# EloDoyard/movie-recommender-system

Hardware: AMD Instinct MI355X
Metric: test-set predictions/sec (kNN k=300, fit+predict+MAE) (higher is better)
Workload: dtype fp16 MFMA similarity filter (fp32 acc) + f64 exact re-rank/prediction

## Files before the change

### movie-recommender-system_amd/csrc/gemm.hip

```cpp
#include <algorithm>
#include <type_traits>
#include <vector>

#include "engine.h"
#include "wave_helpers.h"

namespace knncf {

typedef __attribute__((ext_vector_type(8))) __bf16 bf16x8;
typedef __attribute__((ext_vector_type(8))) _Float16 f16x8;
typedef __attribute__((ext_vector_type(16))) float f32x16;

template <bool F16>
__global__ void k_densify(const int64_t* __restrict__ u_ptr, const int32_t* __restrict__ s_col,
                          const double* __restrict__ s_pre, const int32_t* __restrict__ rows, int32_t row_begin,
                          int32_t n_rows, const int32_t* __restrict__ colmap, bf16_t* __restrict__ panel, int64_t ld, int ones) {
    int32_t wave = (blockIdx.x * blockDim.x + threadIdx.x) >> 6;
    int32_t lane = threadIdx.x & 63;
    if (wave >= n_rows) return;
    int32_t u = rows ? rows[wave] : row_begin + wave;
    int64_t b = u_ptr[u], e = u_ptr[u + 1];
    bf16_t* out = panel + (int64_t)wave * ld;
    for (int64_t p = b + lane; p < e; p += 64) {
        int32_t c = colmap ? colmap[s_col[p]] : s_col[p];
        if (c >= 0) {
            const float x = ones ? 1.0f : (float)s_pre[p];
            if (F16) reinterpret_cast<_Float16*>(out)[c] = (_Float16)x;
            else out[c] = (bf16_t)x;
        }
    }
}

template <bool F16>
__global__ void __launch_bounds__(256) k_densify_rows(const int64_t* __restrict__ u_ptr, const int32_t* __restrict__ s_col,
                                                      const double* __restrict__ s_pre, const int32_t* __restrict__ rows, int32_t row_begin,
                                                      int32_t n_rows, const int32_t* __restrict__ colmap, bf16_t* __restrict__ panel, int64_t ld,
                                                      int ones) {
    extern __shared__ __attribute__((aligned(16))) char smem[];
    const int lane = threadIdx.x & 63;
    const int32_t n_waves = (int32_t)((gridDim.x * blockDim.x) >> 6);
    bf16_t* my = reinterpret_cast<bf16_t*>(smem) + (size_t)(threadIdx.x >> 6) * ld;
    auto wave_sync = [] {
        __builtin_amdgcn_fence(__ATOMIC_ACQ_REL, "wavefront");
        __builtin_amdgcn_wave_barrier();
    };
    for (int32_t wave = (int32_t)((blockIdx.x * blockDim.x + threadIdx.x) >> 6); wave < n_rows; wave += n_waves) {
        for (int64_t c = lane; c < ld / 8; c += 64) reinterpret_cast<uint4*>(my)[c] = make_uint4(0u, 0u, 0u, 0u);
        wave_sync();
        const int32_t u = rows ? rows[wave] : row_begin + wave;
        const int64_t b = u_ptr[u], e = u_ptr[u + 1];
        for (int64_t p0 = b; p0 < e; p0 += 512) {
            int32_t it[8];
            double xv[8];
            int32_t cc[8];
#pragma unroll
            for (int q = 0; q < 8; ++q) {
                const int64_t p = p0 + 64 * q + lane;
                it[q] = p < e ? s_col[p] : -1;
                xv[q] = (p < e && !ones) ? s_pre[p] : 1.0;
            }
#pragma unroll
            for (int q = 0; q < 8; ++q) cc[q] = it[q] < 0 ? -1 : (colmap ? colmap[it[q]] : it[q]);
#pragma unroll
            for (int q = 0; q < 8; ++q) {
                if (cc[q] >= 0) {
                    if (F16) reinterpret_cast<_Float16*>(my)[cc[q]] = (_Float16)(float)xv[q];
                    else my[cc[q]] = (bf16_t)(float)xv[q];
                }
            }
        }
        wave_sync();
        uint4* out = reinterpret_cast<uint4*>(panel + (int64_t)wave * ld);
        for (int64_t c = lane; c < ld / 8; c += 64) out[c] = reinterpret_cast<const uint4*>(my)[c];
        wave_sync();
    }
}

void launch_densify(const Train& tr, const int32_t* d_rows, int32_t row_begin, int32_t n_rows,
                    const int32_t* d_colmap, bf16_t* panel, int64_t ld, int64_t panel_rows, bool fp16, hipStream_t st) {
    const size_t lds = (size_t)4 * (size_t)ld * sizeof(bf16_t);
    if (ld % 64 == 0 && lds <= 64 * 1024) {
        if (panel_rows > n_rows) KN_HIP(hipMemsetAsync(panel + (int64_t)n_rows * ld, 0, (size_t)(panel_rows - n_rows) * ld * sizeof(bf16_t), st));
        if (n_rows <= 0) return;
        const int blocks = (int)std::min<int64_t>(ceil_div((int64_t)n_rows * 64, 256), 256 * 16);
        if (fp16) k_densify_rows<true><<<blocks, 256, lds, st>>>(tr.u_ptr.p, tr.s_col.p, tr.s_pre.p, d_rows, row_begin, n_rows, d_colmap, panel, ld, tr.jaccard ? 1 : 0);
        else k_densify_rows<false><<<blocks, 256, lds, st>>>(tr.u_ptr.p, tr.s_col.p, tr.s_pre.p, d_rows, row_begin, n_rows, d_colmap, panel, ld, tr.jaccard ? 1 : 0);
        KN_HIP(hipGetLastError());
        return;
    }
    KN_HIP(hipMemsetAsync(panel, 0, (size_t)panel_rows * ld * sizeof(bf16_t), st));
    if (n_rows <= 0) return;
    int blocks = (int)ceil_div((int64_t)n_rows * 64, 256);
    if (fp16) k_densify<true><<<blocks, 256, 0, st>>>(tr.u_ptr.p, tr.s_col.p, tr.s_pre.p, d_rows, row_begin, n_rows, d_colmap, panel, ld, tr.jaccard ? 1 : 0);
    else k_densify<false><<<blocks, 256, 0, st>>>(tr.u_ptr.p, tr.s_col.p, tr.s_pre.p, d_rows, row_begin, n_rows, d_colmap, panel, ld, tr.jaccard ? 1 : 0);
    KN_HIP(hipGetLastError());
}

__global__ void k_colmap(int32_t I, int32_t H, const int32_t* __restrict__ pop_item, int32_t* __restrict__ colmap) {
    int32_t j = blockIdx.x * blockDim.x + threadIdx.x;
    if (j >= I) return;
    colmap[pop_item[j]] = j < H ? j : -1;
}

void launch_colmap(const Train& tr, int32_t H, int32_t* d_colmap, hipStream_t st) {
    k_colmap<<<(unsigned)ceil_div(tr.I, 256), 256, 0, st>>>(tr.I, H, tr.pop_item.p, d_colmap);
    KN_HIP(hipGetLastError());
}

static constexpr int BK = 64;

template <int ROWS>
struct TileGeom {
    static constexpr int TILE_BYTES = ROWS * BK * 2;
    static constexpr int STAGE_BYTES = 2 * TILE_BYTES;
};

template <int ROWS, int WAVES>
__device__ __forceinline__ void stage_tile(const bf16_t* __restrict__ g, int64_t ld, char* lds_tile, int wave, int lane) {
    constexpr int LOADS = ROWS / 8 / WAVES;
#pragma unroll
    for (int j = 0; j < LOADS; ++j) {
        int piece = wave * LOADS + j;
        int row = piece * 8 + (lane >> 3);
        int slot = lane & 7;
        int chunk = slot ^ ((row >> 1) & 7);
        const bf16_t* src = g + (int64_t)row * ld + chunk * 8;
        __builtin_amdgcn_global_load_lds(src, (__attribute__((address_space(3))) void*)(lds_tile + piece * 1024), 16, 0, 0);
    }
}

__device__ __forceinline__ bf16x8 read_frag(const char* lds_tile, int row, int chunk) {
    int slot = chunk ^ ((row >> 1) & 7);
    return *reinterpret_cast<const bf16x8*>(lds_tile + row * 128 + slot * 16);
}

template <bool F16>
__device__ __forceinline__ f32x16 mfma(bf16x8 a, bf16x8 b, f32x16 c) {
    if (F16) return __builtin_amdgcn_mfma_f32_32x32x16_f16(__builtin_bit_cast(f16x8, a), __builtin_bit_cast(f16x8, b), c, 0, 0, 0);
    return __builtin_amdgcn_mfma_f32_32x32x16_bf16(a, b, c, 0, 0, 0);
}

struct EpiGeom {
    static constexpr int WM = 4, WN = 2, WAVES_M = 2, WAVES_N = 4, TB = 256;
    static constexpr int ESZ = (int)sizeof(float);
    static constexpr int IPP = WM / 2;
    static constexpr int PASS_ROWS = IPP * 32;
    static constexpr int PASSES = WAVES_M * (WM / IPP);
    static constexpr int RS = TB * ESZ + 16;
    static constexpr int IMAGE_N = PASS_ROWS * RS;
    static constexpr int RS_T = PASS_ROWS * ESZ + 16;
    static constexpr int IMAGE_T = TB * RS_T;
    static constexpr int IMAGE = IMAGE_N > IMAGE_T ? IMAGE_N : IMAGE_T;
    static constexpr int STAGE = TileGeom<TB>::STAGE_BYTES;
    static constexpr int PAD = IMAGE > STAGE ? ((IMAGE - STAGE + 1023) / 1024) * 1024 : 0;
    static constexpr int SMEM = 2 * STAGE + 2 * PAD;
};

template <bool F16, bool SYM>
__global__ void __launch_bounds__(EpiGeom::WAVES_M * EpiGeom::WAVES_N * 64)
k_gemm_nt_bf16(const bf16_t* __restrict__ A, const bf16_t* __restrict__ B, float* __restrict__ C, int tiles_m,
               int tiles_n, int k_tiles, int64_t lda, int64_t ldb, int64_t ldc, const uint32_t* __restrict__ tile_list, int n_listed) {
    typedef EpiGeom EG;
    constexpr int WM = EG::WM, WN = EG::WN, WAVES_N = EG::WAVES_N, WAVES = EG::WAVES_M * EG::WAVES_N, TB = EG::TB;
    constexpr int TILE_BYTES = TileGeom<TB>::TILE_BYTES, STAGE_BYTES = TileGeom<TB>::STAGE_BYTES;
    constexpr int LOADS_PER_STAGE = 2 * (TB / 8 / WAVES);
    static_assert(LOADS_PER_STAGE == 8, "the counted vmcnt below assumes 8 LDS-DMA instructions per wave per stage");
    extern __shared__ __attribute__((aligned(1024))) char lds[];
    char* const ring = lds + EG::PAD;

    const int nwg = SYM ? n_listed : tiles_m * tiles_n;
    const int xcd = blockIdx.x & 7, q = nwg >> 3, r = nwg & 7;
    const int xcd_first = xcd < r ? xcd * (q + 1) : r * (q + 1) + (xcd - r) * q;
    const int xcd_end = xcd_first + (xcd < r ? q + 1 : q);
    const int stride = ((int)gridDim.x - xcd + 7) >> 3;
    int t = xcd_first + ((int)blockIdx.x >> 3);
    if (t >= xcd_end) return;

    const int lane = threadIdx.x & 63;
    const int wave = threadIdx.x >> 6;
    const int wr = wave / WAVES_N, wc = wave % WAVES_N;
    const int frow = lane & 31;
    const int fhalf = lane >> 5;

    auto tile_of = [&](int wg, int& tm, int& tn) {
        if (SYM) {
            const uint32_t packed = tile_list[wg];
            tm = (int)(packed & 0xffffu);
            tn = (int)(packed >> 16);
            return;
        }
        const int GROUP = 8;
        const int group_sz = GROUP * tiles_n;
        const int gid = wg / group_sz;
        const int first_m = gid * GROUP;
        const int gm = min(GROUP, tiles_m - first_m);
        tm = first_m + (wg % group_sz) % gm;
        tn = (wg % group_sz) / gm;
    };

    int tm, tn;
    tile_of(t, tm, tn);
    const bf16_t* Ag = A + (int64_t)tm * TB * lda;
    const bf16_t* Bg = B + (int64_t)tn * TB * ldb;
    stage_tile<TB, WAVES>(Ag, lda, ring, wave, lane);
    stage_tile<TB, WAVES>(Bg, ldb, ring + TILE_BYTES, wave, lane);
    int slot = 0;
    bool landed = false;

    for (;;) {
        const int t_next = t + stride;
        const bool more = t_next < xcd_end;
        int tm2 = 0, tn2 = 0;
        if (more) tile_of(t_next, tm2, tn2);
        const bf16_t* Ag2 = A + (int64_t)tm2 * TB * lda;
        const bf16_t* Bg2 = B + (int64_t)tn2 * TB * ldb;

        f32x16 acc[WM][WN];
#pragma unroll
        for (int i = 0; i < WM; ++i)
#pragma unroll
            for (int j = 0; j < WN; ++j)
#pragma unroll
                for (int e = 0; e < 16; ++e) acc[i][j][e] = 0.f;

        for (int kt = 0; kt < k_tiles; ++kt) {
            char* cur = ring + slot * STAGE_BYTES;
            char* nxt = ring + (slot ^ 1) * STAGE_BYTES;
            const bool in_tile = kt + 1 < k_tiles;
            if (in_tile) {
                stage_tile<TB, WAVES>(Ag + (int64_t)(kt + 1) * BK, lda, nxt, wave, lane);
                stage_tile<TB, WAVES>(Bg + (int64_t)(kt + 1) * BK, ldb, nxt + TILE_BYTES, wave, lane);
            } else if (more) {
                stage_tile<TB, WAVES>(Ag2, lda, nxt, wave, lane);
                stage_tile<TB, WAVES>(Bg2, ldb, nxt + TILE_BYTES, wave, lane);
            }
            if (!landed) {
                if (in_tile || more) asm volatile("s_waitcnt vmcnt(8)" ::: "memory");
                else asm volatile("s_waitcnt vmcnt(0)" ::: "memory");
            }
            landed = false;
            __builtin_amdgcn_s_barrier();
            asm volatile("" ::: "memory");
#pragma unroll
            for (int ks = 0; ks < BK / 16; ++ks) {
                bf16x8 a[WM];
#pragma unroll
                for (int i = 0; i < WM; ++i) a[i] = read_frag(cur, wr * (WM * 32) + i * 32 + frow, ks * 2 + fhalf);
                bf16x8 b[WN];
#pragma unroll
                for (int j = 0; j < WN; ++j) b[j] = read_frag(cur + TILE_BYTES, wc * (WN * 32) + j * 32 + frow, ks * 2 + fhalf);
#pragma unroll
                for (int i = 0; i < WM; ++i)
#pragma unroll
                    for (int j = 0; j < WN; ++j)
                        acc[i][j] = mfma<F16>(b[j], a[i], acc[i][j]);
            }
            asm volatile("s_waitcnt lgkmcnt(0)" ::: "memory");
            __builtin_amdgcn_s_barrier();
            asm volatile("" ::: "memory");
            slot ^= 1;
        }

        {
            asm volatile("s_waitcnt vmcnt(0)" ::: "memory");
            landed = more;
            constexpr int ESZ = EG::ESZ, RS = EG::RS, IPP = EG::IPP, PASS_ROWS = EG::PASS_ROWS, PASSES = EG::PASSES;
            constexpr int CH = TB * ESZ / 16;
            char* const img = (slot ^ 1) ? ring + STAGE_BYTES : lds;
#pragma unroll
            for (int pass = 0; pass < PASSES; ++pass) {
                const int wrp = pass / (WM / IPP), i0 = (pass % (WM / IPP)) * IPP;
                if (wr == wrp) {
#pragma unroll
                    for (int ii = 0; ii < IPP; ++ii)
#pragma unroll
                        for (int j = 0; j < WN; ++j)
#pragma unroll
                            for (int g = 0; g < 4; ++g) {
                                const int i = i0 + ii;
                                char* dst = img + (ii * 32 + frow) * RS + (wc * (WN * 32) + j * 32 + 8 * g + 4 * fhalf) * ESZ;
                                *reinterpret_cast<float4*>(dst) = make_float4(acc[i][j][4 * g], acc[i][j][4 * g + 1], acc[i][j][4 * g + 2], acc[i][j][4 * g + 3]);
                            }
                }
                __syncthreads();
                float* Cg = C + ((int64_t)tm * TB + wrp * (WM * 32) + i0 * 32) * ldc + (int64_t)tn * TB;
                for (int idx = threadIdx.x; idx < PASS_ROWS * CH; idx += WAVES * 64) {
                    const int row = idx / CH, ch = idx - row * CH;
                    const uint4 v = *reinterpret_cast<const uint4*>(img + row * RS + ch * 16);
                    typedef __attribute__((ext_vector_type(4))) uint32_t u32x4;
                    __builtin_nontemporal_store(__builtin_bit_cast(u32x4, v), reinterpret_cast<u32x4*>(reinterpret_cast<char*>(Cg + (int64_t)row * ldc) + ch * 16));
                }
                __syncthreads();
                if (SYM && tm != tn) {
                    constexpr int RS_T = EG::RS_T;
                    constexpr int CHT = PASS_ROWS * ESZ / 16;
                    if (wr == wrp) {
#pragma unroll
                        for (int ii = 0; ii < IPP; ++ii)
#pragma unroll
                            for (int j = 0; j < WN; ++j)
#pragma unroll
                                for (int g = 0; g < 4; ++g)
#pragma unroll
                                    for (int e = 0; e < 4; ++e) {
                                        const int i = i0 + ii;
                                        const int col = wc * (WN * 32) + j * 32 + 8 * g + 4 * fhalf + e;
                                        float* dst = reinterpret_cast<float*>(img + col * RS_T) + (ii * 32 + frow);
                                        *dst = acc[i][j][4 * g + e];
                                    }
                    }
                    __syncthreads();
                    float* Ct = C + (int64_t)tn * TB * ldc + (int64_t)tm * TB + wrp * (WM * 32) + i0 * 32;
                    for (int idx = threadIdx.x; idx < TB * CHT; idx += WAVES * 64) {
                        const int row = idx / CHT, ch = idx - row * CHT;
                        const uint4 v = *reinterpret_cast<const uint4*>(img + row * RS_T + ch * 16);
                        typedef __attribute__((ext_vector_type(4))) uint32_t u32x4;
                        __builtin_nontemporal_store(__builtin_bit_cast(u32x4, v), reinterpret_cast<u32x4*>(reinterpret_cast<char*>(Ct + (int64_t)row * ldc) + ch * 16));
                    }
                    __syncthreads();
                }
            }
        }
        if (!more) break;
        t = t_next;
        tm = tm2;
        tn = tn2;
        Ag = Ag2;
        Bg = Bg2;
    }
}

template <int ROWS, int WAVES>
__device__ __forceinline__ void stage_tile_u(const bf16_t* g_uniform, uint32_t ld2, char* lds_tile, int wave, uint32_t voff) {
    constexpr int LOADS = ROWS / 8 / WAVES;
    static_assert(LOADS % 2 == 0, "pieces alternate between even and odd");
    const char* base = reinterpret_cast<const char*>(uniform_ptr(g_uniform));
#ifdef KNNCF_OV_ABL_NOLOAD
    return;
#endif
#pragma unroll
    for (int j = 0; j < LOADS; ++j) {
        const int piece = wave * LOADS + j;
        const char* src = base + (uint64_t)((uint32_t)piece * 8u * ld2) + (uint64_t)((j & 1) ? (voff ^ 64u) : voff);
        __builtin_amdgcn_global_load_lds(reinterpret_cast<const bf16_t*>(src), (__attribute__((address_space(3))) void*)(lds_tile + piece * 1024), 16, 0, 0);
    }
}

#ifdef KNNCF_OV_ABL_NOSTORE
#define KN_OV_STORE "s_nop 0 ; "
#define KN_OV_STORES 0
#else
#define KN_OV_STORE
#define KN_OV_STORES 4
#endif
template <bool F16, bool SYM, bool SPREAD>
__global__ void __launch_bounds__(512)
k_gemm_nt_ov(const bf16_t* __restrict__ A, const bf16_t* __restrict__ B, _Float16* __restrict__ C, int tiles_m, int tiles_n,
             int k_tiles, int64_t lda, int64_t ldb, int64_t ldc, const uint32_t* __restrict__ tile_list, int n_listed, float clamp_hi) {
    constexpr int WM = 4, WN = 2, WAVES_N = 4, WAVES = 8, TB = 256;
    constexpr int TILE_BYTES = TileGeom<TB>::TILE_BYTES, STAGE_BYTES = TileGeom<TB>::STAGE_BYTES;
    constexpr int LOADS_PER_STAGE = 2 * (TB / 8 / WAVES);
    static_assert(LOADS_PER_STAGE == 8, "the counted waits below assume 8 LDS-DMA instructions per wave per stage");
    extern __shared__ __attribute__((aligned(1024))) char lds[];
    char* const ring = lds;

    const int nwg = SYM ? n_listed : tiles_m * tiles_n;
    const int xcd = blockIdx.x & 7, q = nwg >> 3, r = nwg & 7;
    const int xcd_first = xcd < r ? xcd * (q + 1) : r * (q + 1) + (xcd - r) * q;
    const int xcd_end = xcd_first + (xcd < r ? q + 1 : q);
    const int stride = ((int)gridDim.x - xcd + 7) >> 3;
    int t = xcd_first + ((int)blockIdx.x >> 3);
    if (t >= xcd_end) return;

    const int lane = threadIdx.x & 63;
    const int wave = threadIdx.x >> 6;
    const int wr = wave / WAVES_N, wc = wave % WAVES_N;
    const int frow = lane & 31, fhalf = lane >> 5;
    char* const stg = lds + 2 * STAGE_BYTES + wave * 4096;
    const int uwave = __builtin_amdgcn_readfirstlane(wave);
    const uint32_t lda2 = (uint32_t)lda * 2u, ldb2 = (uint32_t)ldb * 2u;
    const uint32_t sw16 = (uint32_t)(((lane & 7) ^ (lane >> 4)) * 16);
    uint32_t voff_a = (uint32_t)(lane >> 3) * lda2 + sw16, voff_b = (uint32_t)(lane >> 3) * ldb2 + sw16;
    asm volatile("" : "+v"(voff_a), "+v"(voff_b));

    auto tile_of = [&](int wg, int& tm, int& tn) {
        if (SYM) {
            const uint32_t packed = tile_list[wg];
            tm = (int)(packed & 0xffffu);
            tn = (int)(packed >> 16);
            return;
        }
        const int GROUP = 8;
        const int group_sz = GROUP * tiles_n;
        const int gid = wg / group_sz;
        const int first_m = gid * GROUP;
        const int gm = min(GROUP, tiles_m - first_m);
        tm = first_m + (wg % group_sz) % gm;
        tn = (wg % group_sz) / gm;
    };

    typedef __attribute__((ext_vector_type(2))) _Float16 h2;
    typedef __attribute__((ext_vector_type(4))) uint32_t u32x4;
    constexpr int NP = 2, UNITS = 4;
    uint32_t P[NP][WN][8];
#pragma unroll
    for (int i = 0; i < NP; ++i)
#pragma unroll
        for (int j = 0; j < WN; ++j)
#pragma unroll
            for (int h = 0; h < 8; ++h) P[i][j][h] = 0u;
    int ptm = 0, ptn = 0;
    int unit = 1000;

    const uint32_t ldc2 = (uint32_t)ldc * 2u;
    const uint32_t vo_n = (uint32_t)(lane >> 3) * ldc2 + (uint32_t)(lane & 7) * 16u;
    const uint32_t stg_a = (uint32_t)(uintptr_t)(__attribute__((address_space(3))) char*)stg;
    const uint32_t aw_n = stg_a + ((uint32_t)frow * 128u | (uint32_t)fhalf * 8u | (uint32_t)(frow & 7) * 16u);
    const uint32_t lr_n = (uint32_t)(lane >> 3) * 128u + (uint32_t)(((lane & 7) ^ (lane >> 3)) * 16);
    const uint32_t lra_n = stg_a + lr_n, lra_t = stg_a + (uint32_t)lane * 16u;
    const uint32_t aw_m = stg_a + (uint32_t)fhalf * 512u + (uint32_t)frow * 2u;
    const uint32_t so_1 = (uint32_t)__builtin_amdgcn_readfirstlane((int)(8u * ldc2));
    auto drain_normal = [&](const uint32_t (&R)[WN][8], int I) -> int {
        u32x4 q0, q1, q2, q3;
        uint32_t tmp_a;
        _Float16* Cg = C + ((int64_t)ptm * TB + wr * (WM * 32) + I * 32) * ldc + (int64_t)ptn * TB + wc * (WN * 32);
        const uint64_t cb = reinterpret_cast<uint64_t>(uniform_ptr(Cg));
        const u32x4 rs = {(uint32_t)cb, (uint32_t)(cb >> 32) & 0xffffu, 0x7fffffffu, 0x00020000u};
        asm volatile(
                "v_xor_b32 %[t], 0, %[aw]\n\tds_write2_b32 %[t], %[r00], %[r01] offset1:1\n\t"
                "v_xor_b32 %[t], 16, %[aw]\n\tds_write2_b32 %[t], %[r02], %[r03] offset1:1\n\t"
                "v_xor_b32 %[t], 32, %[aw]\n\tds_write2_b32 %[t], %[r04], %[r05] offset1:1\n\t"
                "v_xor_b32 %[t], 48, %[aw]\n\tds_write2_b32 %[t], %[r06], %[r07] offset1:1\n\t"
                "v_xor_b32 %[t], 64, %[aw]\n\tds_write2_b32 %[t], %[r10], %[r11] offset1:1\n\t"
                "v_xor_b32 %[t], 80, %[aw]\n\tds_write2_b32 %[t], %[r12], %[r13] offset1:1\n\t"
                "v_xor_b32 %[t], 96, %[aw]\n\tds_write2_b32 %[t], %[r14], %[r15] offset1:1\n\t"
                "v_xor_b32 %[t], 112, %[aw]\n\tds_write2_b32 %[t], %[r16], %[r17] offset1:1\n\t"
                "ds_read_b128 %[q0], %[lr] offset:0\n\t"
                "ds_read_b128 %[q1], %[lr] offset:1024\n\t"
                "ds_read_b128 %[q2], %[lr] offset:2048\n\t"
                "ds_read_b128 %[q3], %[lr] offset:3072\n\t"
                "s_waitcnt lgkmcnt(3)\n\t" KN_OV_STORE "buffer_store_dwordx4 %[q0], %[vo], %[rs], %[so0] offen nt\n\t"
                "s_waitcnt lgkmcnt(2)\n\t" KN_OV_STORE "buffer_store_dwordx4 %[q1], %[vo], %[rs], %[so1] offen nt\n\t"
                "s_waitcnt lgkmcnt(1)\n\t" KN_OV_STORE "buffer_store_dwordx4 %[q2], %[vo], %[rs], %[so2] offen nt\n\t"
                "s_waitcnt lgkmcnt(0)\n\t" KN_OV_STORE "buffer_store_dwordx4 %[q3], %[vo], %[rs], %[so3] offen nt\n\t"
                "s_nop 1"
            : [t] "=&v"(tmp_a), [q0] "=&v"(q0), [q1] "=&v"(q1), [q2] "=&v"(q2), [q3] "=&v"(q3)
            : [aw] "v"(aw_n), [lr] "v"(lra_n), [vo] "v"(vo_n), [rs] "s"(rs), [so0] "s"(0u), [so1] "s"(so_1), [so2] "s"(2u * so_1), [so3] "s"(3u * so_1),
              [r00] "v"(R[0][0]), [r01] "v"(R[0][1]), [r02] "v"(R[0][2]), [r03] "v"(R[0][3]), [r04] "v"(R[0][4]), [r05] "v"(R[0][5]), [r06] "v"(R[0][6]), [r07] "v"(R[0][7]), [r10] "v"(R[1][0]), [r11] "v"(R[1][1]), [r12] "v"(R[1][2]), [r13] "v"(R[1][3]), [r14] "v"(R[1][4]), [r15] "v"(R[1][5]), [r16] "v"(R[1][6]), [r17] "v"(R[1][7])
            : "memory");
        return KN_OV_STORES;
    };
    auto drain_mirror = [&](const uint32_t (&Ra)[WN][8], const uint32_t (&Rb)[WN][8], int pr, auto J_) -> int {
        constexpr int J = decltype(J_)::value;
        if (!SYM || ptm == ptn) return 0;
        u32x4 q0, q1, q2, q3;
        _Float16* Ct = C + ((int64_t)ptn * TB + wc * (WN * 32) + J * 32) * ldc + (int64_t)ptm * TB + wr * (WM * 32) + pr * 64;
        const uint64_t cb = reinterpret_cast<uint64_t>(uniform_ptr(Ct));
        const u32x4 rs = {(uint32_t)cb, (uint32_t)(cb >> 32) & 0xffffu, 0x7fffffffu, 0x00020000u};
        asm volatile(
                "ds_write_b16 %[aw], %[r00] offset:0\n\tds_write_b16_d16_hi %[aw], %[r00] offset:128\n\t"
                "ds_write_b16 %[aw], %[r01] offset:256\n\tds_write_b16_d16_hi %[aw], %[r01] offset:384\n\t"
                "ds_write_b16 %[aw], %[r02] offset:1024\n\tds_write_b16_d16_hi %[aw], %[r02] offset:1152\n\t"
                "ds_write_b16 %[aw], %[r03] offset:1280\n\tds_write_b16_d16_hi %[aw], %[r03] offset:1408\n\t"
                "ds_write_b16 %[aw], %[r04] offset:2048\n\tds_write_b16_d16_hi %[aw], %[r04] offset:2176\n\t"
                "ds_write_b16 %[aw], %[r05] offset:2304\n\tds_write_b16_d16_hi %[aw], %[r05] offset:2432\n\t"
                "ds_write_b16 %[aw], %[r06] offset:3072\n\tds_write_b16_d16_hi %[aw], %[r06] offset:3200\n\t"
                "ds_write_b16 %[aw], %[r07] offset:3328\n\tds_write_b16_d16_hi %[aw], %[r07] offset:3456\n\t"
                "ds_write_b16 %[aw], %[r10] offset:64\n\tds_write_b16_d16_hi %[aw], %[r10] offset:192\n\t"
                "ds_write_b16 %[aw], %[r11] offset:320\n\tds_write_b16_d16_hi %[aw], %[r11] offset:448\n\t"
                "ds_write_b16 %[aw], %[r12] offset:1088\n\tds_write_b16_d16_hi %[aw], %[r12] offset:1216\n\t"
                "ds_write_b16 %[aw], %[r13] offset:1344\n\tds_write_b16_d16_hi %[aw], %[r13] offset:1472\n\t"
                "ds_write_b16 %[aw], %[r14] offset:2112\n\tds_write_b16_d16_hi %[aw], %[r14] offset:2240\n\t"
                "ds_write_b16 %[aw], %[r15] offset:2368\n\tds_write_b16_d16_hi %[aw], %[r15] offset:2496\n\t"
                "ds_write_b16 %[aw], %[r16] offset:3136\n\tds_write_b16_d16_hi %[aw], %[r16] offset:3264\n\t"
                "ds_write_b16 %[aw], %[r17] offset:3392\n\tds_write_b16_d16_hi %[aw], %[r17] offset:3520\n\t"
                "ds_read_b128 %[q0], %[lr] offset:0\n\t"
                "ds_read_b128 %[q1], %[lr] offset:1024\n\t"
                "ds_read_b128 %[q2], %[lr] offset:2048\n\t"
                "ds_read_b128 %[q3], %[lr] offset:3072\n\t"
                "s_waitcnt lgkmcnt(3)\n\t" KN_OV_STORE "buffer_store_dwordx4 %[q0], %[vo], %[rs], %[so0] offen nt\n\t"
                "s_waitcnt lgkmcnt(2)\n\t" KN_OV_STORE "buffer_store_dwordx4 %[q1], %[vo], %[rs], %[so1] offen nt\n\t"
                "s_waitcnt lgkmcnt(1)\n\t" KN_OV_STORE "buffer_store_dwordx4 %[q2], %[vo], %[rs], %[so2] offen nt\n\t"
                "s_waitcnt lgkmcnt(0)\n\t" KN_OV_STORE "buffer_store_dwordx4 %[q3], %[vo], %[rs], %[so3] offen nt\n\t"
                "s_nop 1"
            : [q0] "=&v"(q0), [q1] "=&v"(q1), [q2] "=&v"(q2), [q3] "=&v"(q3)
            : [aw] "v"(aw_m), [lr] "v"(lra_t), [vo] "v"(vo_n), [rs] "s"(rs), [so0] "s"(0u), [so1] "s"(so_1), [so2] "s"(2u * so_1), [so3] "s"(3u * so_1),
              [r00] "v"(Ra[J][0]), [r01] "v"(Ra[J][1]), [r02] "v"(Ra[J][2]), [r03] "v"(Ra[J][3]), [r04] "v"(Ra[J][4]), [r05] "v"(Ra[J][5]), [r06] "v"(Ra[J][6]), [r07] "v"(Ra[J][7]), [r10] "v"(Rb[J][0]), [r11] "v"(Rb[J][1]), [r12] "v"(Rb[J][2]), [r13] "v"(Rb[J][3]), [r14] "v"(Rb[J][4]), [r15] "v"(Rb[J][5]), [r16] "v"(Rb[J][6]), [r17] "v"(Rb[J][7])
            : "memory");
        return KN_OV_STORES;
    };
    auto drain_unit = [&](int u) -> int {
        switch (u) {
            case 0: return drain_normal(P[0], 2);
            case 1: return drain_normal(P[1], 3);
            case 2: return drain_mirror(P[0], P[1], 1, std::integral_constant<int, 0>{});
            default: return drain_mirror(P[0], P[1], 1, std::integral_constant<int, 1>{});
        }
    };

#ifdef KNNCF_OV_ABL_HOTLOAD
#define KN_OV_ROW(x) 0
#else
#define KN_OV_ROW(x) (x)
#endif
    int tm, tn;
    tile_of(t, tm, tn);
    const bf16_t* Ag = A + (int64_t)KN_OV_ROW(tm) * TB * lda;
    const bf16_t* Bg = B + (int64_t)KN_OV_ROW(tn) * TB * ldb;
    stage_tile_u<TB, WAVES>(Ag, lda2, ring, uwave, voff_a);
    stage_tile_u<TB, WAVES>(Bg, ldb2, ring + TILE_BYTES, uwave, voff_b);
    int slot = 0;
    uint32_t ops = LOADS_PER_STAGE, mark[2] = {LOADS_PER_STAGE, 0u};
    auto wait_for = [&](int s) {
        const uint32_t allow = ops - mark[s];
        if (allow >= 32) asm volatile("s_waitcnt vmcnt(32)" ::: "memory");
        else if (allow >= 28) asm volatile("s_waitcnt vmcnt(28)" ::: "memory");
        else if (allow >= 24) asm volatile("s_waitcnt vmcnt(24)" ::: "memory");
        else if (allow >= 20) asm volatile("s_waitcnt vmcnt(20)" ::: "memory");
        else if (allow >= 16) asm volatile("s_waitcnt vmcnt(16)" ::: "memory");
        else if (allow >= 12) asm volatile("s_waitcnt vmcnt(12)" ::: "memory");
        else if (allow >= 8) asm volatile("s_waitcnt vmcnt(8)" ::: "memory");
        else if (allow >= 4) asm volatile("s_waitcnt vmcnt(4)" ::: "memory");
        else asm volatile("s_waitcnt vmcnt(0)" ::: "memory");
    };
    bool pre_issued = false;
    constexpr bool spread = SPREAD;

    for (;;) {
        const int t_next = t + stride;
        const bool more = t_next < xcd_end;
        int tm2 = 0, tn2 = 0;
        if (more) tile_of(t_next, tm2, tn2);
        const bf16_t* Ag2 = A + (int64_t)KN_OV_ROW(tm2) * TB * lda;
        const bf16_t* Bg2 = B + (int64_t)KN_OV_ROW(tn2) * TB * ldb;

        f32x16 acc[WM][WN];
#pragma unroll
        for (int i = 0; i < WM; ++i)
#pragma unroll
            for (int j = 0; j < WN; ++j)
#pragma unroll
                for (int e = 0; e < 16; ++e) acc[i][j][e] = 0.f;

        for (int kt = 0; kt < k_tiles; ++kt) {
            char* cur = ring + slot * STAGE_BYTES;
            char* nxt = ring + (slot ^ 1) * STAGE_BYTES;
            const bool in_tile = kt + 1 < k_tiles;
            if (kt == 0 && pre_issued) {
                pre_issued = false;
            } else if (in_tile) {
                stage_tile_u<TB, WAVES>(Ag + (int64_t)(kt + 1) * BK, lda2, nxt, uwave, voff_a);
                stage_tile_u<TB, WAVES>(Bg + (int64_t)(kt + 1) * BK, ldb2, nxt + TILE_BYTES, uwave, voff_b);
                ops += LOADS_PER_STAGE;
                mark[slot ^ 1] = ops;
            } else if (more) {
                stage_tile_u<TB, WAVES>(Ag2, lda2, nxt, uwave, voff_a);
                stage_tile_u<TB, WAVES>(Bg2, ldb2, nxt + TILE_BYTES, uwave, voff_b);
                ops += LOADS_PER_STAGE;
                mark[slot ^ 1] = ops;
            }
            wait_for(slot);
            __builtin_amdgcn_s_barrier();
            asm volatile("" ::: "memory");
            {
                const char* ca = cur;
                const char* cb = cur + TILE_BYTES;
                const int arow = wr * (WM * 32) + frow, brow = wc * (WN * 32) + frow;
                bf16x8 b0 = read_frag(cb, brow, fhalf), b1 = read_frag(cb, brow + 32, fhalf);
                bf16x8 a_cur = read_frag(ca, arow, fhalf);
                const bool unit_step = !spread || kt >= 2;
#pragma unroll
                for (int ks = 0; ks < BK / 16; ++ks) {
                    bf16x8 b0n = b0, b1n = b1;
#pragma unroll
                    for (int i = 0; i < WM; ++i) {
                        bf16x8 a_next = a_cur;
                        if (i + 1 < WM) {
                            a_next = read_frag(ca, arow + (i + 1) * 32, ks * 2 + fhalf);
                        } else if (ks + 1 < BK / 16) {
                            a_next = read_frag(ca, arow, (ks + 1) * 2 + fhalf);
                            b0n = read_frag(cb, brow, (ks + 1) * 2 + fhalf);
                            b1n = read_frag(cb, brow + 32, (ks + 1) * 2 + fhalf);
                        }
#ifndef KNNCF_OV_ABL_NOMFMA
                        acc[i][0] = mfma<F16>(b0, a_cur, acc[i][0]);
                        acc[i][1] = mfma<F16>(b1, a_cur, acc[i][1]);
#else
                        acc[i][0][0] += (float)a_cur[0] + (float)b0[0];
                        acc[i][1][0] += (float)a_cur[1] + (float)b1[0];
#endif
                        a_cur = a_next;
                    }
                    b0 = b0n;
                    b1 = b1n;
                    if ((ks == 0 || (ks == 2 && !spread)) && unit_step && unit < UNITS) {
                        ops += (uint32_t)drain_unit(unit);
                        ++unit;
                    }
                }
            }
            asm volatile("s_waitcnt lgkmcnt(0)" ::: "memory");
            __builtin_amdgcn_s_barrier();
            asm volatile("" ::: "memory");
            slot ^= 1;
        }
        if (more && k_tiles >= 2) {
            char* nxt = ring + (slot ^ 1) * STAGE_BYTES;
            stage_tile_u<TB, WAVES>(Ag2 + BK, lda2, nxt, uwave, voff_a);
            stage_tile_u<TB, WAVES>(Bg2 + BK, ldb2, nxt + TILE_BYTES, uwave, voff_b);
            ops += LOADS_PER_STAGE;
            mark[slot ^ 1] = ops;
            pre_issued = true;
        }
        while (unit < UNITS) {
            ops += (uint32_t)drain_unit(unit);
            ++unit;
        }
        ptm = tm;
        ptn = tn;
        auto convert = [&](uint32_t (&R)[WN][8], auto I_) {
            constexpr int I = decltype(I_)::value;
#pragma unroll
            for (int j = 0; j < WN; ++j)
#pragma unroll
                for (int h = 0; h < 8; ++h) {
                    h2 v;
                    v[0] = (_Float16)__builtin_amdgcn_fmed3f(acc[I][j][2 * h], -clamp_hi, clamp_hi);
                    v[1] = (_Float16)__builtin_amdgcn_fmed3f(acc[I][j][2 * h + 1], -clamp_hi, clamp_hi);
                    R[j][h] = __builtin_bit_cast(uint32_t, v);
                }
        };
        {
            uint32_t Q0[WN][8], Q1[WN][8];
            convert(Q0, std::integral_constant<int, 0>{});
            ops += (uint32_t)drain_normal(Q0, 0);
            convert(Q1, std::integral_constant<int, 1>{});
            ops += (uint32_t)drain_normal(Q1, 1);
            ops += (uint32_t)drain_mirror(Q0, Q1, 0, std::integral_constant<int, 0>{});
            ops += (uint32_t)drain_mirror(Q0, Q1, 0, std::integral_constant<int, 1>{});
        }
        convert(P[0], std::integral_constant<int, 2>{});
        convert(P[1], std::integral_constant<int, 3>{});
        unit = 0;
        if (!more) break;
        t = t_next;
        tm = tm2;
        tn = tn2;
        Ag = Ag2;
        Bg = Bg2;
    }
    while (unit < UNITS) {
        (void)drain_unit(unit);
        ++unit;
    }
}

template <bool F16, bool SYM, bool SPREAD>
static void launch_gemm_ov_t(const bf16_t* A, const bf16_t* B, _Float16* C, int64_t M, int64_t N, int64_t K, int64_t lda, int64_t ldb,
                           int64_t ldc, const uint32_t* tile_list, int64_t n_listed, bool clamp, hipStream_t st) {
    constexpr int TB = 256;
    constexpr int SMEM = 2 * TileGeom<TB>::STAGE_BYTES + 8 * 4096;
    static_assert(SMEM <= 160 * 1024, "gemm: LDS plan exceeds the CU's 160 KiB");
    const int64_t tiles = SYM ? n_listed : (M / TB) * (N / TB);
    KN_REQUIRE(tiles > 0 && tiles < (1ll << 31), KNNCF_E_INVALID, "gemm: grid too large");
    static PerDeviceState state;
    const int64_t slots = (int64_t)per_device_at_least(state, 1, [&](size_t) {
        KN_HIP(hipFuncSetAttribute((const void*)k_gemm_nt_ov<F16, SYM, SPREAD>, hipFuncAttributeMaxDynamicSharedMemorySize, SMEM));
        int dev = 0, cus = 0;
        KN_HIP(hipGetDevice(&dev));
        KN_HIP(hipDeviceGetAttribute(&cus, hipDeviceAttributeMultiprocessorCount, dev));
        return (size_t)std::max(1, cus);
    });
    const unsigned grid = (unsigned)(tiles < slots ? tiles : slots);
    k_gemm_nt_ov<F16, SYM, SPREAD><<<grid, 512, SMEM, st>>>(A, B, C, (int)(M / TB), (int)(N / TB), (int)(K / BK), lda, ldb, ldc, tile_list,
                                                    (int)n_listed, clamp ? 1.0f : 65504.0f);
    KN_HIP(hipGetLastError());
}

template <bool F16, bool SYM>
static void launch_gemm_ov(const bf16_t* A, const bf16_t* B, _Float16* C, int64_t M, int64_t N, int64_t K, int64_t lda, int64_t ldb,
                           int64_t ldc, const uint32_t* tile_list, int64_t n_listed, bool clamp, hipStream_t st) {
    if (K / BK >= 6) launch_gemm_ov_t<F16, SYM, true>(A, B, C, M, N, K, lda, ldb, ldc, tile_list, n_listed, clamp, st);
    else launch_gemm_ov_t<F16, SYM, false>(A, B, C, M, N, K, lda, ldb, ldc, tile_list, n_listed, clamp, st);
}

template <bool F16, bool SYM>
static void launch_gemm_f32(const bf16_t* A, const bf16_t* B, float* C, int64_t M, int64_t N, int64_t K, int64_t lda, int64_t ldb,
                            int64_t ldc, const uint32_t* tile_list, int64_t n_listed, hipStream_t st) {
    constexpr int TB = EpiGeom::TB, THREADS = EpiGeom::WAVES_M * EpiGeom::WAVES_N * 64, SMEM = EpiGeom::SMEM;
    static_assert(SMEM <= 160 * 1024, "gemm: LDS plan exceeds the CU's 160 KiB");
    const int64_t tiles = SYM ? n_listed : (M / TB) * (N / TB);
    KN_REQUIRE(tiles > 0 && tiles < (1ll << 31), KNNCF_E_INVALID, "gemm: grid too large");
    static PerDeviceState state;
    const int64_t slots = (int64_t)per_device_at_least(state, 1, [&](size_t) {
        KN_HIP(hipFuncSetAttribute((const void*)k_gemm_nt_bf16<F16, SYM>, hipFuncAttributeMaxDynamicSharedMemorySize, SMEM));
        int dev = 0, cus = 0, per_cu = 0;
        KN_HIP(hipGetDevice(&dev));
        KN_HIP(hipDeviceGetAttribute(&cus, hipDeviceAttributeMultiprocessorCount, dev));
        KN_HIP(hipOccupancyMaxActiveBlocksPerMultiprocessor(&per_cu, k_gemm_nt_bf16<F16, SYM>, THREADS, SMEM));
        return (size_t)std::max(1, cus * (per_cu > 0 ? per_cu : 1));
    });
    const unsigned grid = (unsigned)(tiles < slots ? tiles : slots);
    k_gemm_nt_bf16<F16, SYM><<<grid, THREADS, SMEM, st>>>(A, B, C, (int)(M / TB), (int)(N / TB), (int)(K / BK), lda, ldb, ldc, tile_list,
                                                          (int)n_listed);
    KN_HIP(hipGetLastError());
}

void launch_gemm_nt(const bf16_t* A, const bf16_t* B, void* C, bool c_fp16, int64_t M, int64_t N, int64_t K, int64_t lda,
                    int64_t ldb, int64_t ldc, bool fp16, bool clamp, hipStream_t st) {
    KN_REQUIRE(M % 256 == 0 && N % 256 == 0 && K % BK == 0 && K > 0, KNNCF_E_INVALID, "gemm: shape not tile-aligned");
    KN_REQUIRE(lda % 8 == 0 && ldb % 8 == 0, KNNCF_E_INVALID, "gemm: leading dimensions must be multiples of 8");
    if (c_fp16 && fp16) launch_gemm_ov<true, false>(A, B, static_cast<_Float16*>(C), M, N, K, lda, ldb, ldc, nullptr, 0, clamp, st);
    else if (c_fp16) launch_gemm_ov<false, false>(A, B, static_cast<_Float16*>(C), M, N, K, lda, ldb, ldc, nullptr, 0, clamp, st);
    else if (fp16) launch_gemm_f32<true, false>(A, B, static_cast<float*>(C), M, N, K, lda, ldb, ldc, nullptr, 0, st);
    else launch_gemm_f32<false, false>(A, B, static_cast<float*>(C), M, N, K, lda, ldb, ldc, nullptr, 0, st);
}

void gemm_sym_tile_list(int32_t n_tiles, std::vector<uint32_t>& out) {
    constexpr int32_t GROUP = 8;
    out.clear();
    out.reserve((size_t)n_tiles * (n_tiles + 1) / 2);
    for (int32_t g = 0; g < n_tiles; g += GROUP)
        for (int32_t tn = g; tn < n_tiles; ++tn)
            for (int32_t tm = g; tm < std::min(g + GROUP, n_tiles) && tm <= tn; ++tm) out.push_back((uint32_t)tm | ((uint32_t)tn << 16));
}

void launch_gemm_sym(const bf16_t* B, void* C, bool c_fp16, int64_t N, int64_t K, int64_t ldb, int64_t ldc, bool fp16, bool clamp,
                     const uint32_t* d_tile_list, int64_t n_listed, hipStream_t st) {
    KN_REQUIRE(N % 256 == 0 && N / 128 < 65536 && K % BK == 0 && K > 0 && ldb % 8 == 0 && ldc % 8 == 0, KNNCF_E_INVALID, "symmetric gemm: shape not tile-aligned");
    if (c_fp16 && fp16) launch_gemm_ov<true, true>(B, B, static_cast<_Float16*>(C), N, N, K, ldb, ldb, ldc, d_tile_list, n_listed, clamp, st);
    else if (c_fp16) launch_gemm_ov<false, true>(B, B, static_cast<_Float16*>(C), N, N, K, ldb, ldb, ldc, d_tile_list, n_listed, clamp, st);
    else if (fp16) launch_gemm_f32<true, true>(B, B, static_cast<float*>(C), N, N, K, ldb, ldb, ldc, d_tile_list, n_listed, st);
    else launch_gemm_f32<false, true>(B, B, static_cast<float*>(C), N, N, K, ldb, ldb, ldc, d_tile_list, n_listed, st);
}

}
```

Measured before the change: 88.38 million.

## Rewrite GEMM mainloop with explicit ds_read pipelining, single barrier, and wave priority

```diff
diff --git a/movie-recommender-system_amd/csrc/gemm.hip b/movie-recommender-system_amd/csrc/gemm.hip
--- a/movie-recommender-system_amd/csrc/gemm.hip
+++ b/movie-recommender-system_amd/csrc/gemm.hip
@@ -359,8 +359,6 @@
              int k_tiles, int64_t lda, int64_t ldb, int64_t ldc, const uint32_t* __restrict__ tile_list, int n_listed, float clamp_hi) {
     constexpr int WM = 4, WN = 2, WAVES_N = 4, WAVES = 8, TB = 256;
     constexpr int TILE_BYTES = TileGeom<TB>::TILE_BYTES, STAGE_BYTES = TileGeom<TB>::STAGE_BYTES;
-    constexpr int LOADS_PER_STAGE = 2 * (TB / 8 / WAVES);
-    static_assert(LOADS_PER_STAGE == 8, "the counted waits below assume 8 LDS-DMA instructions per wave per stage");
     extern __shared__ __attribute__((aligned(1024))) char lds[];
     char* const ring = lds;
 
@@ -505,34 +503,47 @@
 #endif
     int tm, tn;
     tile_of(t, tm, tn);
-    const bf16_t* Ag = A + (int64_t)KN_OV_ROW(tm) * TB * lda;
-    const bf16_t* Bg = B + (int64_t)KN_OV_ROW(tn) * TB * ldb;
-    stage_tile_u<TB, WAVES>(Ag, lda2, ring, uwave, voff_a);
-    stage_tile_u<TB, WAVES>(Bg, ldb2, ring + TILE_BYTES, uwave, voff_b);
     int slot = 0;
-    uint32_t ops = LOADS_PER_STAGE, mark[2] = {LOADS_PER_STAGE, 0u};
-    auto wait_for = [&](int s) {
-        const uint32_t allow = ops - mark[s];
-        if (allow >= 32) asm volatile("s_waitcnt vmcnt(32)" ::: "memory");
-        else if (allow >= 28) asm volatile("s_waitcnt vmcnt(28)" ::: "memory");
-        else if (allow >= 24) asm volatile("s_waitcnt vmcnt(24)" ::: "memory");
-        else if (allow >= 20) asm volatile("s_waitcnt vmcnt(20)" ::: "memory");
-        else if (allow >= 16) asm volatile("s_waitcnt vmcnt(16)" ::: "memory");
-        else if (allow >= 12) asm volatile("s_waitcnt vmcnt(12)" ::: "memory");
-        else if (allow >= 8) asm volatile("s_waitcnt vmcnt(8)" ::: "memory");
-        else if (allow >= 4) asm volatile("s_waitcnt vmcnt(4)" ::: "memory");
-        else asm volatile("s_waitcnt vmcnt(0)" ::: "memory");
+    int s_t = t, s_kt = 0;
+    const bf16_t* s_A = A + (int64_t)KN_OV_ROW(tm) * TB * lda;
+    const bf16_t* s_B = B + (int64_t)KN_OV_ROW(tn) * TB * ldb;
+    auto stage_next = [&](int s) {
+        if (s_t >= xcd_end) return;
+        char* dst = ring + s * STAGE_BYTES;
+        stage_tile_u<TB, WAVES>(s_A + (int64_t)s_kt * BK, lda2, dst, uwave, voff_a);
+        stage_tile_u<TB, WAVES>(s_B + (int64_t)s_kt * BK, ldb2, dst + TILE_BYTES, uwave, voff_b);
+        if (++s_kt < k_tiles) return;
+        s_kt = 0;
+        s_t += stride;
+        if (s_t >= xcd_end) return;
+        int sm, sn;
+        tile_of(s_t, sm, sn);
+        s_A = A + (int64_t)KN_OV_ROW(sm) * TB * lda;
+        s_B = B + (int64_t)KN_OV_ROW(sn) * TB * ldb;
     };
-    bool pre_issued = false;
     constexpr bool spread = SPREAD;
+
+    stage_next(0);
+    stage_next(1);
+    asm volatile("s_waitcnt vmcnt(0)" ::: "memory");
+    __builtin_amdgcn_s_barrier();
+    asm volatile("" ::: "memory");
+    if (uwave >= WAVES / 2) __builtin_amdgcn_s_setprio(1);
+
+    const uint32_t ring_a = (uint32_t)(uintptr_t)(__attribute__((address_space(3))) char*)ring;
+    const uint32_t fr_lane = (uint32_t)frow * 128u + (uint32_t)((fhalf ^ ((frow >> 1) & 7)) * 16);
+    const uint32_t fr_a = ring_a + (uint32_t)wr * (WM * 32 * 128) + fr_lane;
+    const uint32_t fr_b = ring_a + TILE_BYTES + (uint32_t)wc * (WN * 32 * 128) + fr_lane;
+    bf16x8 a[WM], bq[2][WN];
+#define KN_FRAG_READ(f, addr, off) asm volatile("ds_read_b128 %0, %1 offset:" #off : "=v"(f) : "v"(addr) : "memory")
+#define KN_FRAG_WAIT1(n, x) asm volatile("s_waitcnt lgkmcnt(" #n ")" : "+v"(x) : : "memory")
+#define KN_FRAG_WAIT3(n, x, y, z) asm volatile("s_waitcnt lgkmcnt(" #n ")" : "+v"(x), "+v"(y), "+v"(z) : : "memory")
 
     for (;;) {
         const int t_next = t + stride;
         const bool more = t_next < xcd_end;
         int tm2 = 0, tn2 = 0;
         if (more) tile_of(t_next, tm2, tn2);
-        const bf16_t* Ag2 = A + (int64_t)KN_OV_ROW(tm2) * TB * lda;
-        const bf16_t* Bg2 = B + (int64_t)KN_OV_ROW(tn2) * TB * ldb;
 
         f32x16 acc[WM][WN];
 #pragma unroll
@@ -541,79 +552,98 @@
             for (int j = 0; j < WN; ++j)
 #pragma unroll
                 for (int e = 0; e < 16; ++e) acc[i][j][e] = 0.f;
+#ifdef KNNCF_OV_ABL_NOMFMA
+        float abl_sink = 0.f;
+#endif
 
         for (int kt = 0; kt < k_tiles; ++kt) {
-            char* cur = ring + slot * STAGE_BYTES;
-            char* nxt = ring + (slot ^ 1) * STAGE_BYTES;
-            const bool in_tile = kt + 1 < k_tiles;
-            if (kt == 0 && pre_issued) {
-                pre_issued = false;
-            } else if (in_tile) {
-                stage_tile_u<TB, WAVES>(Ag + (int64_t)(kt + 1) * BK, lda2, nxt, uwave, voff_a);
-                stage_tile_u<TB, WAVES>(Bg + (int64_t)(kt + 1) * BK, ldb2, nxt + TILE_BYTES, uwave, voff_b);
-                ops += LOADS_PER_STAGE;
-                mark[slot ^ 1] = ops;
-            } else if (more) {
-                stage_tile_u<TB, WAVES>(Ag2, lda2, nxt, uwave, voff_a);
-                stage_tile_u<TB, WAVES>(Bg2, ldb2, nxt + TILE_BYTES, uwave, voff_b);
-                ops += LOADS_PER_STAGE;
-                mark[slot ^ 1] = ops;
+            const uint32_t ca = fr_a + (uint32_t)slot * STAGE_BYTES, cb = fr_b + (uint32_t)slot * STAGE_BYTES;
+            const uint32_t na = fr_a + (uint32_t)(slot ^ 1) * STAGE_BYTES, nb = fr_b + (uint32_t)(slot ^ 1) * STAGE_BYTES;
+            const bool last = kt + 1 == k_tiles;
+            const bool unit_step = !spread || kt >= 2;
+            if (kt == 0) {
+                KN_FRAG_READ(bq[0][0], cb, 0);
+                KN_FRAG_READ(bq[0][1], cb, 4096);
+                KN_FRAG_READ(a[0], ca, 0);
+                KN_FRAG_READ(a[1], ca, 4096);
+                KN_FRAG_READ(a[2], ca, 8192);
+                KN_FRAG_READ(a[3], ca, 12288);
             }
-            wait_for(slot);
-            __builtin_amdgcn_s_barrier();
-            asm volatile("" ::: "memory");
+            auto pair = [&](auto KS_, auto I_) {
+                constexpr int ks = decltype(KS_)::value, i = decltype(I_)::value;
+#ifndef KNNCF_OV_ABL_NOMFMA
+                acc[i][0] = mfma<F16>(bq[ks & 1][0], a[i], acc[i][0]);
+                acc[i][1] = mfma<F16>(bq[ks & 1][1], a[i], acc[i][1]);
+#else
+                (void)i;
+                abl_sink += (float)a[i][0] + (float)bq[ks & 1][0][0] + (float)bq[ks & 1][1][0];
+#endif
+            };
+            auto substep = [&](auto KS_) {
+                constexpr int ks = decltype(KS_)::value;
+                const uint32_t xa = ca ^ (uint32_t)((ks + 1) * 32), xb = cb ^ (uint32_t)((ks + 1) * 32);
+                KN_FRAG_READ(bq[(ks + 1) & 1][0], xb, 0);
+                KN_FRAG_READ(bq[(ks + 1) & 1][1], xb, 4096);
+                __builtin_amdgcn_sched_barrier(0);
+                KN_FRAG_WAIT3(5, bq[ks & 1][0], bq[ks & 1][1], a[0]);
+                pair(KS_, std::integral_constant<int, 0>{});
+                KN_FRAG_READ(a[0], xa, 0);
+                __builtin_amdgcn_sched_barrier(0);
+                KN_FRAG_WAIT1(5, a[1]);
+                pair(KS_, std::integral_constant<int, 1>{});
+                KN_FRAG_READ(a[1], xa, 4096);
+                __builtin_amdgcn_sched_barrier(0);
+                KN_FRAG_WAIT1(5, a[2]);
+                pair(KS_, std::integral_constant<int, 2>{});
+                KN_FRAG_READ(a[2], xa, 8192);
+                __builtin_amdgcn_sched_barrier(0);
+                KN_FRAG_WAIT1(5, a[3]);
+                pair(KS_, std::integral_constant<int, 3>{});
+                KN_FRAG_READ(a[3], xa, 12288);
+                __builtin_amdgcn_sched_barrier(0);
+                if ((ks == 0 || (ks == 2 && !spread)) && unit_step && unit < UNITS) {
+                    (void)drain_unit(unit);
+                    ++unit;
+                }
+            };
+            substep(std::integral_constant<int, 0>{});
+            substep(std::integral_constant<int, 1>{});
+            substep(std::integral_constant<int, 2>{});
             {
-                const char* ca = cur;
-                const char* cb = cur + TILE_BYTES;
-                const int arow = wr * (WM * 32) + frow, brow = wc * (WN * 32) + frow;
-                bf16x8 b0 = read_frag(cb, brow, fhalf), b1 = read_frag(cb, brow + 32, fhalf);
-                bf16x8 a_cur = read_frag(ca, arow, fhalf);
-                const bool unit_step = !spread || kt >= 2;
-#pragma unroll
-                for (int ks = 0; ks < BK / 16; ++ks) {
-                    bf16x8 b0n = b0, b1n = b1;
-#pragma unroll
-                    for (int i = 0; i < WM; ++i) {
-                        bf16x8 a_next = a_cur;
-                        if (i + 1 < WM) {
-                            a_next = read_frag(ca, arow + (i + 1) * 32, ks * 2 + fhalf);
-                        } else if (ks + 1 < BK / 16) {
-                            a_next = read_frag(ca, arow, (ks + 1) * 2 + fhalf);
-                            b0n = read_frag(cb, brow, (ks + 1) * 2 + fhalf);
-                            b1n = read_frag(cb, brow + 32, (ks + 1) * 2 + fhalf);
-                        }
-#ifndef KNNCF_OV_ABL_NOMFMA
-                        acc[i][0] = mfma<F16>(b0, a_cur, acc[i][0]);
-                        acc[i][1] = mfma<F16>(b1, a_cur, acc[i][1]);
-#else
-                        acc[i][0][0] += (float)a_cur[0] + (float)b0[0];
-                        acc[i][1][0] += (float)a_cur[1] + (float)b1[0];
+                typedef std::integral_constant<int, 3> K3;
+                static_assert(BK / 16 == 4 && WM == 4 && WN == 2, "the k-step is written out for four k-substeps of four pairs");
+                KN_FRAG_WAIT3(3, bq[1][0], bq[1][1], a[0]);
+                pair(K3{}, std::integral_constant<int, 0>{});
+                __builtin_amdgcn_sched_barrier(0);
+                KN_FRAG_WAIT1(2, a[1]);
+                pair(K3{}, std::integral_constant<int, 1>{});
+                __builtin_amdgcn_sched_barrier(0);
+                asm volatile("s_waitcnt lgkmcnt(0)" : "+v"(a[2]), "+v"(a[3]) : : "memory");
+                asm volatile("s_waitcnt vmcnt(0)" ::: "memory");
+                __builtin_amdgcn_s_barrier();
+                asm volatile("" ::: "memory");
+                stage_next(slot);
+                if (!last) {
+                    KN_FRAG_READ(bq[0][0], nb, 0);
+                    KN_FRAG_READ(bq[0][1], nb, 4096);
+                    KN_FRAG_READ(a[0], na, 0);
+                    KN_FRAG_READ(a[1], na, 4096);
+                }
+                __builtin_amdgcn_sched_barrier(0);
+                pair(K3{}, std::integral_constant<int, 2>{});
+                if (!last) KN_FRAG_READ(a[2], na, 8192);
+                __builtin_amdgcn_sched_barrier(0);
+                pair(K3{}, std::integral_constant<int, 3>{});
+                if (!last) KN_FRAG_READ(a[3], na, 12288);
+                __builtin_amdgcn_sched_barrier(0);
+            }
+            slot ^= 1;
+        }
+#ifdef KNNCF_OV_ABL_NOMFMA
+        acc[0][0][0] += abl_sink;
 #endif
-                        a_cur = a_next;
-                    }
-                    b0 = b0n;
-                    b1 = b1n;
-                    if ((ks == 0 || (ks == 2 && !spread)) && unit_step && unit < UNITS) {
-                        ops += (uint32_t)drain_unit(unit);
-                        ++unit;
-                    }
-                }
-            }
-            asm volatile("s_waitcnt lgkmcnt(0)" ::: "memory");
-            __builtin_amdgcn_s_barrier();
-            asm volatile("" ::: "memory");
-            slot ^= 1;
-        }
-        if (more && k_tiles >= 2) {
-            char* nxt = ring + (slot ^ 1) * STAGE_BYTES;
-            stage_tile_u<TB, WAVES>(Ag2 + BK, lda2, nxt, uwave, voff_a);
-            stage_tile_u<TB, WAVES>(Bg2 + BK, ldb2, nxt + TILE_BYTES, uwave, voff_b);
-            ops += LOADS_PER_STAGE;
-            mark[slot ^ 1] = ops;
-            pre_issued = true;
-        }
         while (unit < UNITS) {
-            ops += (uint32_t)drain_unit(unit);
+            (void)drain_unit(unit);
             ++unit;
         }
         ptm = tm;
@@ -633,11 +663,11 @@
         {
             uint32_t Q0[WN][8], Q1[WN][8];
             convert(Q0, std::integral_constant<int, 0>{});
-            ops += (uint32_t)drain_normal(Q0, 0);
+            (void)drain_normal(Q0, 0);
             convert(Q1, std::integral_constant<int, 1>{});
-            ops += (uint32_t)drain_normal(Q1, 1);
-            ops += (uint32_t)drain_mirror(Q0, Q1, 0, std::integral_constant<int, 0>{});
-            ops += (uint32_t)drain_mirror(Q0, Q1, 0, std::integral_constant<int, 1>{});
+            (void)drain_normal(Q1, 1);
+            (void)drain_mirror(Q0, Q1, 0, std::integral_constant<int, 0>{});
+            (void)drain_mirror(Q0, Q1, 0, std::integral_constant<int, 1>{});
         }
         convert(P[0], std::integral_constant<int, 2>{});
         convert(P[1], std::integral_constant<int, 3>{});
@@ -646,8 +676,6 @@
         t = t_next;
         tm = tm2;
         tn = tn2;
-        Ag = Ag2;
-        Bg = Bg2;
     }
     while (unit < UNITS) {
         (void)drain_unit(unit);
```

Result: faster. 89.58 million (median of 6 runs) (+1.4%).
